# ekimb/rust-mdbg

Measured on AMD Instinct MI355X. Metric: Gbases/s ingested to k-min-mer graph, higher is better.
Workload: dtype u64

## Files before the change

### rust_mdbg_amd/csrc/table.hip

```cpp
#include "mdbg_dev.h"

struct __attribute__((aligned(32))) Slot {
    u64 word;
    u64 m1;
    u64 m2;
    u32 count;
    u32 pad;
};
constexpr u64 EMPTY = ~0ull;
constexpr u64 HMUL = 0x9E3779B97F4A7C15ull;

struct KeySrc {
    const u64* mh;
    const u64* arena;
    u32 k;
};

__device__ inline u64 load_relaxed(const u64* p) { return __hip_atomic_load(p, __ATOMIC_RELAXED, __HIP_MEMORY_SCOPE_AGENT); }

__device__ inline u64 rep_elem(const KeySrc& ks, u64 word, u32 j) {
    const u32 rep = (u32)word;
    if (word & (1ull << 33)) return ks.arena[(u64)rep * (ks.k + 2) + j];
    return (word & (1ull << 32)) ? ks.mh[(u64)rep + ks.k - 1 - j] : ks.mh[(u64)rep + j];
}

__device__ inline bool window_reversed(const u64* __restrict__ w, u32 k) {
    for (u32 j = 0; j < k / 2 + 1 && j < k; ++j) {
        const u64 a = w[j], b = w[k - 1 - j];
        if (a < b) return false;
        if (a > b) return true;
    }
    return true;
}
template <class ElemFn>
__device__ inline u64 key_hash_fn(ElemFn elem, u32 k) {
    u64 h0 = 0x243F6A8885A308D3ull, h1 = 0x13198A2E03707344ull, h2 = 0xA4093822299F31D0ull, h3 = 0x082EFA98EC4E6C89ull;
    u32 j = 0;
    for (; j + 4 <= k; j += 4) {
        h0 = (h0 ^ elem(j)) * HMUL;     h0 ^= h0 >> 29;
        h1 = (h1 ^ elem(j + 1)) * HMUL; h1 ^= h1 >> 29;
        h2 = (h2 ^ elem(j + 2)) * HMUL; h2 ^= h2 >> 29;
        h3 = (h3 ^ elem(j + 3)) * HMUL; h3 ^= h3 >> 29;
    }
    if (j < k) { h0 = (h0 ^ elem(j)) * HMUL; h0 ^= h0 >> 29; }
    if (j + 1 < k) { h1 = (h1 ^ elem(j + 1)) * HMUL; h1 ^= h1 >> 29; }
    if (j + 2 < k) { h2 = (h2 ^ elem(j + 2)) * HMUL; h2 ^= h2 >> 29; }
    return fmix64(h0 ^ rol64(h1, 17) ^ rol64(h2, 31) ^ rol64(h3, 47));
}
__device__ inline u64 key_hash_window(const u64* __restrict__ w, u32 k, bool rev) {
    return key_hash_fn([&](u32 j) { return rev ? w[k - 1 - j] : w[j]; }, k);
}
__device__ inline u64 key_hash_window_hbm(const u64* __restrict__ w, u32 k, bool rev, u64& smallest) {
    u64 h[4] = {0x243F6A8885A308D3ull, 0x13198A2E03707344ull, 0xA4093822299F31D0ull, 0x082EFA98EC4E6C89ull};
    const u64* const p = rev ? w + (k - 1) : w;
    const long st = rev ? -1 : 1;
    u64 mn = ~0ull;
    for (u32 j0 = 0; j0 < k; j0 += 16) {
        u64 v[16];
#pragma unroll
        for (int t = 0; t < 16; ++t) { const u32 j = j0 + t < k ? j0 + t : k - 1; v[t] = p[st * (long)j]; }
#pragma unroll
        for (int t = 0; t < 16; ++t)
            if (j0 + t < k) { h[t & 3] = (h[t & 3] ^ v[t]) * HMUL; h[t & 3] ^= h[t & 3] >> 29; mn = v[t] < mn ? v[t] : mn; }
    }
    smallest = mn;
    return fmix64(h[0] ^ rol64(h[1], 17) ^ rol64(h[2], 31) ^ rol64(h[3], 47));
}
__device__ inline u64 key_hash_canon(const u64* __restrict__ key, u32 k) {
    return key_hash_fn([&](u32 j) { return key[j]; }, k);
}

struct TableArgs {
    Slot* tab; u64 cap;
    u64* mx;
    u32 A;
    u64* n_distinct;
    KeySrc ks;
    u32 own_world, own_rank;
    const u64* own_thr;
    u32* probe_err;
    u64* own_inserted;
    u64 fp_mask;
    unsigned long long* link_ctr;
    u32 no_chain;
    u8* claim;
};

__device__ inline u64 home_slot(u64 h, u64 cap) { return __umul64hi(h << 24, cap); }

__device__ inline void push_ordinal(const TableArgs& T, u64 s, u64 x) {
    Slot* e = T.tab + s;
    const u32 A = T.A;
    const u64* last = A == 1 ? &e->m1 : A == 2 ? &e->m2 : &T.mx[s * (A - 2) + (A - 3)];
    if (x > load_relaxed(last)) return;
    u64 carry = x;
    for (u32 lvl = 0; lvl < A && carry != EMPTY; ++lvl) {
        u64* m = lvl == 0 ? &e->m1 : lvl == 1 ? &e->m2 : &T.mx[s * (A - 2) + (lvl - 2)];
        const u64 old = atomicMin((unsigned long long*)m, (unsigned long long)carry);
        if (old > carry) carry = old;
    }
}

template <class EqFn>
__device__ inline u64 upsert_slot_from(const TableArgs& T, u64 h, u64 myword_lo, EqFn same_key, bool& claimed, u64 s, u64 probes);
template <class EqFn>
__device__ inline u64 upsert_slot(const TableArgs& T, u64 h, u64 myword_lo, EqFn same_key, bool& claimed) {
    return upsert_slot_from(T, h, myword_lo, same_key, claimed, home_slot(h, T.cap), 0);
}
template <class EqFn>
__device__ inline u64 upsert_slot_from(const TableArgs& T, u64 h, u64 myword_lo, EqFn same_key, bool& claimed, u64 s, u64 probes) {
    claimed = false;
    const u64 fp = (h >> 34) & T.fp_mask;
    const u64 myword = (fp << 34) | myword_lo;
    for (; probes <= T.cap; ++probes) {
        u64 w = load_relaxed(&T.tab[s].word);
        if (w == EMPTY) {
            const u64 old = atomicCAS((unsigned long long*)&T.tab[s].word, (unsigned long long)EMPTY, (unsigned long long)myword);
            if (old == EMPTY) { wave_agg_inc(T.n_distinct); claimed = true; return s; }
            w = old;
        }
        if ((w >> 34) == fp && same_key(w)) return s;
        s = s + 1 == T.cap ? 0 : s + 1;
    }
    *T.probe_err = 1;
    return ~0ull;
}
typedef u64 u64x2_a8 __attribute__((ext_vector_type(2), aligned(8)));
__device__ inline bool same_key_window(const KeySrc& ks, u64 w, const u64* wl, bool rev_mine) {
    const u32 k = ks.k, rep = (u32)w;
    const u64* rp; bool cross;
    if (w & (1ull << 33)) { rp = ks.arena + (u64)rep * (k + 2); cross = rev_mine; }
    else { rp = ks.mh + rep; cross = rev_mine != ((w & (1ull << 32)) != 0); }
    if (k < 8) {
        u64 diff = 0;
        for (u32 j = 0; j < k; ++j) diff |= rp[j] ^ wl[cross ? k - 1 - j : j];
        return !diff;
    }
    if (k >= 16) {
        for (u32 j = 0;; j += 16) {
            if (j + 16 > k) j = k - 16;
            u64x2_a8 a[8];
#pragma unroll
            for (int t = 0; t < 8; ++t) a[t] = *(const u64x2_a8*)(rp + j + 2 * t);
            u64 diff = 0;
            if (!cross) {
                const u64* m = wl + j;
#pragma unroll
                for (int t = 0; t < 8; ++t) diff |= (a[t].x ^ m[2 * t]) | (a[t].y ^ m[2 * t + 1]);
            } else {
                const u64* m = wl + (k - 16 - j);
#pragma unroll
                for (int t = 0; t < 8; ++t) diff |= (a[t].x ^ m[15 - 2 * t]) | (a[t].y ^ m[14 - 2 * t]);
            }
            if (diff) return false;
            if (j + 16 >= k) return true;
        }
    }
    for (u32 j = 0;; j += 8) {
        if (j + 8 > k) j = k - 8;
        const u64x2_a8 a0 = *(const u64x2_a8*)(rp + j), a1 = *(const u64x2_a8*)(rp + j + 2),
                       a2 = *(const u64x2_a8*)(rp + j + 4), a3 = *(const u64x2_a8*)(rp + j + 6);
        u64 diff;
        if (!cross) {
            const u64* m = wl + j;
            diff = (a0.x ^ m[0]) | (a0.y ^ m[1]) | (a1.x ^ m[2]) | (a1.y ^ m[3]) | (a2.x ^ m[4]) | (a2.y ^ m[5]) | (a3.x ^ m[6]) | (a3.y ^ m[7]);
        } else {
            const u64* m = wl + (k - 8 - j);
            diff = (a0.x ^ m[7]) | (a0.y ^ m[6]) | (a1.x ^ m[5]) | (a1.y ^ m[4]) | (a2.x ^ m[3]) | (a2.y ^ m[2]) | (a3.x ^ m[1]) | (a3.y ^ m[0]);
        }
        if (diff) return false;
        if (j + 8 >= k) return true;
    }
}

constexpr u32 OWNER_BINS = 65536, OWNER_THR_AT = 1, OWNER_TAB_AT = 64, OWNER_PARAM_WORDS = OWNER_TAB_AT + OWNER_BINS / 8;
struct OwnerSpec { u32 world; const u64* thr; };
__device__ inline u32 owner_of_min(u64 m, u32 k, OwnerSpec os);
__device__ inline u32 window_owner(const u64* __restrict__ w, u32 k, OwnerSpec os) {
    if (os.world <= 1) return 0;
    u64 m = w[0];
    for (u32 j = 1; j < k; ++j) { const u64 x = w[j]; m = x < m ? x : m; }
    return owner_of_min(m, k, os);
}
__device__ inline u32 owner_of_min(u64 m, u32 k, OwnerSpec os) {
    (void)k;
    if (os.world <= 1) return 0;
    if (!os.thr) return (u32)__umul64hi(fmix64(m), (u64)os.world);
    const u64 mul = os.thr[0];
    if (mul) {
        const u64 bin = __umul64hi(m, mul);
        const u32 o = ((const u8*)(os.thr + OWNER_TAB_AT))[bin < OWNER_BINS ? bin : OWNER_BINS - 1];
        return o < os.world ? o : os.world - 1;
    }
    const u64* const thr = os.thr + OWNER_THR_AT;
    u32 lo = 0, hi = os.world - 1;
    while (lo < hi) { const u32 mid = (lo + hi) >> 1; if (thr[mid] <= m) lo = mid + 1; else hi = mid; }
    return lo;
}
__global__ void owner_thresholds_kernel(double bound, u32 k, u32 world, u64* __restrict__ thr) {
    const u32 r = threadIdx.x + 1;
    if (threadIdx.x == 0) thr[0] = 0;
    thr += OWNER_THR_AT;
    if (r >= world) return;
    const double x = -expm1(log1p(-(double)r / (double)world) / (double)k);
    double v = x * bound;
    thr[r - 1] = v >= 18446744073709549568.0 ? ~0ull : (u64)v;
}
void launch_owner_thresholds(double bound, u32 k, u32 world, u64* thr, hipStream_t s) {
    if (world > 1) hipLaunchKernelGGL(owner_thresholds_kernel, dim3(1), dim3(64), 0, s, bound, k, world, thr);
}

struct OwnerCodes { u64 mul; const u64* thr; u32 world; };
__device__ inline OwnerCodes owner_codes_of(OwnerSpec os) { OwnerCodes c; c.thr = os.thr; c.world = os.world; c.mul = os.thr ? os.thr[0] : 0; return c; }
__device__ inline u16 owner_code(u64 v, const OwnerCodes& c) {
    if (c.mul) { const u64 bin = __umul64hi(v, c.mul); return (u16)(bin < OWNER_BINS ? bin : OWNER_BINS - 1); }
    const u64* const thr = c.thr + OWNER_THR_AT;
    u32 lo = 0, hi = c.world - 1;
    while (lo < hi) { const u32 mid = (lo + hi) >> 1; if (thr[mid] <= v) lo = mid + 1; else hi = mid; }
    return (u16)lo;
}
__device__ inline u32 owner_of_code(u16 code, const OwnerCodes& c) {
    if (!c.mul) return code;
    const u32 o = ((const u8*)(c.thr + OWNER_TAB_AT))[code];
    return o < c.world ? o : c.world - 1;
}
template <class ValueFn, class ValidFn>
__device__ inline const u16* span_min_codes(ValueFn value, ValidFn valid, u32 nv, u32 k, const OwnerCodes& c, u16* a, u16* b, u32& p) {
    for (u32 t = threadIdx.x; t < nv; t += 256) a[t] = valid(t) ? owner_code(value(t), c) : (u16)0xFFFFu;
    __syncthreads();
    for (p = 1; 2 * p <= k; p *= 2) {
        for (u32 t = threadIdx.x; t < nv; t += 256) { const u16 x = a[t], y = t + p < nv ? a[t + p] : (u16)0xFFFFu; b[t] = x < y ? x : y; }
        __syncthreads();
        u16* const sw = a; a = b; b = sw;
    }
    return a;
}

__device__ inline u64 upsert_wave_h(const TableArgs& T, bool act, u32 li, u64 i, const u64* w, u32 k, bool rev, u64 h, bool& claimed, bool& found);
__device__ inline u64 upsert_wave(const TableArgs& T, bool act, u32 li, u64 i, const u64* w, u32 k, bool& claimed, bool& found) {
    bool rev = false; u64 h = 0;
    if (act) { rev = window_reversed(w, k); h = key_hash_window(w, k, rev); }
    return upsert_wave_h(T, act, li, i, w, k, rev, h, claimed, found);
}
__device__ inline u64 upsert_wave_h(const TableArgs& T, bool act, u32 li, u64 i, const u64* w, u32 k, bool rev, u64 h, bool& claimed, bool& found) {
    const int lane = threadIdx.x & 63;
    const u64 fp = (h >> 34) & T.fp_mask;
    const u64 myword_lo = ((u64)rev << 32) | (u64)(u32)i;
    auto eq = [&](u64 word) { return same_key_window(T.ks, word, w, rev); };
    u64 s = act ? home_slot(h, T.cap) : 0, word = EMPTY, probes = 0;
    claimed = false;
    bool cand = false;
    if (act) {
        for (; probes <= T.cap; ++probes) {
            u64 wv = load_relaxed(&T.tab[s].word);
            if (wv == EMPTY) {
                const u64 old = atomicCAS((unsigned long long*)&T.tab[s].word, (unsigned long long)EMPTY, (unsigned long long)((fp << 34) | myword_lo));
                if (old == EMPTY) { wave_agg_inc(T.n_distinct); claimed = true; break; }
                wv = old;
            }
            if ((wv >> 34) == fp) { word = wv; cand = true; break; }
            s = s + 1 == T.cap ? 0 : s + 1;
        }
        if (!claimed && !cand) { *T.probe_err = 1; s = ~0ull; }
    }
    const bool cross = rev != ((word & (1ull << 32)) != 0);
    const u32 rep = (u32)word;
    const u32 p_li = (u32)__shfl_up((int)li, 1, 64), p_rep = (u32)__shfl_up((int)rep, 1, 64);
    const int p_info = __shfl_up((int)((cand && !(word & (1ull << 33)) ? 1 : 0) | (cross ? 2 : 0)), 1, 64);
    const bool link = cand && !T.no_chain && lane > 0 && !(word & (1ull << 33)) && (p_info & 1) && p_li + 1 == li && ((p_info >> 1) & 1) == (int)cross &&
                      rep == (cross ? p_rep - 1u : p_rep + 1u);
    bool pass = false;
    if (cand) pass = link ? T.ks.mh[(u64)rep + (cross ? 0u : k - 1u)] == w[k - 1] : eq(word);
    const u64 heads = __ballot(!link), fails = __ballot(cand && !pass);
    found = pass;
    if (link && pass) {
        const int hp = 63 - __clzll((unsigned long long)(heads & ((2ull << lane) - 1ull)));
        found = ((fails >> hp) & ((2ull << (lane - hp)) - 1ull)) == 0;
    }
    if (T.link_ctr) { const u64 lm = __ballot(link && found); if (lane == 0 && lm) atomicAdd(T.link_ctr, (unsigned long long)__popcll(lm)); }
    if (cand && !found) {
        const bool skip = !link;
        s = upsert_slot_from(T, h, myword_lo, eq, claimed, skip ? (s + 1 == T.cap ? 0 : s + 1) : s, probes + (skip ? 1 : 0));
        found = !claimed && s != ~0ull;
    }
    return s;
}

constexpr int OWN_SPAN = 2048;
__global__ __launch_bounds__(256) void insert_windows_kernel(TableArgs T, const u64* __restrict__ mh, const u32* __restrict__ mread,
                                                                   const u64* __restrict__ roff, u64 i0, u64 i1, u32 slot0, u64 first_ordinal,
                                                                   u32* __restrict__ cap_err, const u64* __restrict__ i1_dev, u64 n_lim) {
    extern __shared__ u64 sh_keys[];
    if (cap_err[1]) return;
    if (i1_dev) { i1 = *i1_dev; if (i0 + (u64)blockIdx.x * OWN_SPAN >= i1) return; }
    const u32 k = T.ks.k;
    u16* const list = (u16*)(sh_keys + OWN_SPAN + k);
    u32* const n_own = (u32*)(list + OWN_SPAN);
    u8* const cl = (u8*)(n_own + 4);
    const u64 b0 = i0 + (u64)blockIdx.x * OWN_SPAN;
    const u64 lim = b0 + OWN_SPAN + k - 1 < i1 ? b0 + OWN_SPAN + k - 1 : i1;
    for (u64 t = b0 + threadIdx.x; t < lim; t += 256) sh_keys[t - b0] = mh[t];
    if (threadIdx.x == 0) *n_own = 0;
    if (T.claim) for (int u = threadIdx.x; u < OWN_SPAN / 8; u += 256) ((u64*)cl)[u] = 0;
    __syncthreads();
    const bool by_codes = T.own_world > 1 && T.own_thr != nullptr;
    const u16* mc = nullptr; u32 pc = 1; OwnerCodes oc{};
    if (by_codes) {
        u16* const ca = (u16*)(cl + OWN_SPAN);
        oc = owner_codes_of(OwnerSpec{T.own_world, T.own_thr});
        const u32 n_st = (u32)(lim - b0);
        mc = span_min_codes([&](u32 t) { return sh_keys[t]; }, [&](u32 t) { return t < n_st; }, OWN_SPAN + k - 1, k, oc, ca, ca + (OWN_SPAN + k), pc);
    }
#pragma unroll
    for (int u = 0; u < OWN_SPAN / 256; ++u) {
        const u32 li = u * 256 + threadIdx.x;
        const u64 i = b0 + li;
        bool mine = false;
        bool own = i + k <= i1;
        if (own && T.own_world > 1) {
            if (by_codes) { const u16 x = mc[li], y = mc[li + k - pc]; own = owner_of_code(x < y ? x : y, oc) == T.own_rank; }
            else own = window_owner(sh_keys + li, k, OwnerSpec{T.own_world, T.own_thr}) == T.own_rank;
        }
        if (own) {
            const u32 slot = mread[i];
            const u64 rs = roff[slot], re = roff[slot + 1];
            mine = re - rs > k && i + k <= re;
        }
        const u64 m = __ballot(mine);
        u32 base = 0;
        if ((threadIdx.x & 63) == 0 && m) base = atomicAdd(n_own, (u32)__popcll(m));
        base = __shfl(base, 0, 64);
        if (mine) list[base + __popcll(m & ((1ull << (threadIdx.x & 63)) - 1))] = (u16)li;
    }
    __syncthreads();
    const u32 n = *n_own;
    if (threadIdx.x == 0 && n && T.own_world > 1) atomicAdd((unsigned long long*)ctr_shard(T.own_inserted), (unsigned long long)n);
    for (u32 j0 = 0; j0 < n; j0 += 256) {
        const u32 j = j0 + threadIdx.x;
        bool act = j < n;
        const u32 li = act ? list[j] : 0u;
        const u64 i = b0 + li;
        u64 ord = 0;
        if (act) {
            const u32 slot = mread[i];
            const u64 win = i - roff[slot];
            if (win > WIN_MASK) { *cap_err = 1; act = false; }
            ord = ((first_ordinal + (slot - slot0)) << WIN_BITS) | win;
        }
        bool claimed, found;
        const u64 s = upsert_wave(T, act, li, i, sh_keys + li, k, claimed, found);
        if (claimed && T.claim) cl[li] = 1;
        if (found) {
            atomicAdd(&T.tab[s].count, 1u);
            push_ordinal(T, s, ord);
        }
    }
    if (T.claim) {
        __syncthreads();
        const u64 hi = i1 - b0 < (u64)OWN_SPAN ? i1 - b0 : (u64)OWN_SPAN;
        for (u32 li = threadIdx.x; li < hi && li < n_lim - (u64)blockIdx.x * OWN_SPAN; li += 256) T.claim[b0 + li] = cl[li];
    }
}

constexpr int OWNL_SPAN = 2048;
constexpr u32 OWNL_MAX_WORLD = 64;
struct OwnerBases { u64 b[OWNL_MAX_WORLD]; };
__device__ inline bool window_starts_at(const u32* __restrict__ mread, const u64* __restrict__ roff, u64 i, u64 i1, u32 k) {
    if (i >= i1) return false;
    const u32 slot = mread[i];
    const u64 rs = roff[slot], re = roff[slot + 1];
    return re - rs > k && i + k <= re;
}
constexpr u32 OWNL_LDS_MAX_K = 1024;
__global__ __launch_bounds__(256) void owner_bins_kernel(const u64* __restrict__ mh, const u32* __restrict__ mread, const u64* __restrict__ roff, u64 i0, u64 i1, u32 k, u64 mul,
                                                         unsigned long long* __restrict__ hist) {
    extern __shared__ u64 sh_min[];
    const u64 b0 = i0 + (u64)blockIdx.x * OWNL_SPAN;
    const bool staged = k <= OWNL_LDS_MAX_K;
    OwnerCodes oc{}; oc.mul = mul;
    const u16* cur = nullptr; u32 p = 1;
    if (staged) { u16* const ca = (u16*)sh_min; cur = span_min_codes([&](u32 t) { return mh[b0 + t]; }, [&](u32 t) { return b0 + t < i1; }, OWNL_SPAN + k - 1, k, oc, ca, ca + (OWNL_SPAN + k), p); }
    const int lane = threadIdx.x & 63;
#pragma unroll 1
    for (int u = 0; u < OWNL_SPAN / 256; ++u) {
        const u32 li = u * 256 + threadIdx.x;
        const u64 i = b0 + li;
        u32 bin = 0xFFFFFFFFu;
        if (window_starts_at(mread, roff, i, i1, k)) {
            if (staged) { const u16 x = cur[li], y = cur[li + k - p]; bin = x < y ? x : y; }
            else { u64 m = mh[i]; for (u32 j = 1; j < k; ++j) { const u64 x = mh[i + j]; m = x < m ? x : m; } bin = owner_code(m, oc); }
        }
        for (u64 todo = __ballot(bin != 0xFFFFFFFFu); todo;) {
            const u32 bb = (u32)__shfl((int)bin, __ffsll((unsigned long long)todo) - 1, 64);
            const u64 mm = __ballot(bin == bb);
            if (bin == bb && (mm & ((1ull << lane) - 1)) == 0) atomicAdd(&hist[bb], (unsigned long long)__popcll(mm));
            todo &= ~mm;
        }
    }
}
void launch_owner_bins(const u64* mh, const u32* mread, const u64* roff, u64 i0, u64 i1, u32 k, u64 mul, u64* hist, hipStream_t s) {
    const size_t lds = k <= OWNL_LDS_MAX_K ? 2 * ((size_t)OWNL_SPAN + k) * sizeof(u16) : 0;
    if (i1 > i0) hipLaunchKernelGGL(owner_bins_kernel, dim3((unsigned)((i1 - i0 + OWNL_SPAN - 1) / OWNL_SPAN)), dim3(256), lds, s, mh, mread, roff, i0, i1, k, mul, (unsigned long long*)hist);
}
__global__ __launch_bounds__(256) void owner_list_count_kernel(const u64* __restrict__ mh, const u32* __restrict__ mread, const u64* __restrict__ roff, u64 i0, u64 i1,
                                                               u32 k, u32 world, const u64* thr, u32* __restrict__ blk_cnt, u8* __restrict__ owner_of) {
    extern __shared__ u64 sh_min[];
    __shared__ u32 hist[OWNL_MAX_WORLD];
    if (threadIdx.x < world) hist[threadIdx.x] = 0;
    const u64 b0 = i0 + (u64)blockIdx.x * OWNL_SPAN;
    const OwnerSpec os{world, thr};
    const bool staged = k <= OWNL_LDS_MAX_K && thr != nullptr && world > 1;
    OwnerCodes oc{}; const u16* cur = nullptr; u32 p = 1;
    if (staged) {
        oc = owner_codes_of(os);
        u16* const ca = (u16*)sh_min;
        cur = span_min_codes([&](u32 t) { return mh[b0 + t]; }, [&](u32 t) { return b0 + t < i1; }, OWNL_SPAN + k - 1, k, oc, ca, ca + (OWNL_SPAN + k), p);
    } else __syncthreads();
#pragma unroll
    for (int u = 0; u < OWNL_SPAN / 256; ++u) {
        const u32 li = u * 256 + threadIdx.x;
        const u64 i = b0 + li;
        u32 o = 0xFFu;
        if (window_starts_at(mread, roff, i, i1, k)) {
            if (staged) { const u16 x = cur[li], y = cur[li + k - p]; o = owner_of_code(x < y ? x : y, oc); }
            else o = window_owner(mh + i, k, os);
            atomicAdd(&hist[o], 1u);
        }
        if (i < i1) owner_of[i - i0] = (u8)o;
    }
    __syncthreads();
    if (threadIdx.x < world) blk_cnt[(size_t)blockIdx.x * world + threadIdx.x] = hist[threadIdx.x];
}
__global__ __launch_bounds__(256) void owner_list_write_kernel(const u64* __restrict__ mh, const u32* __restrict__ mread, const u64* __restrict__ roff, u64 i0, u64 i1,
                                                               u32 k, u32 world, const u64* thr, u32 slot0, const u64* __restrict__ blk_off, OwnerBases bases, u32* __restrict__ list,
                                                               const u8* __restrict__ owner_of, u32 direct_owner, u32* __restrict__ direct_dst) {
    constexpr int NG = OWNL_SPAN / 64;
    __shared__ u32 grp[NG][OWNL_MAX_WORLD];
    for (int t = threadIdx.x; t < NG * (int)OWNL_MAX_WORLD; t += 256) ((u32*)grp)[t] = 0;
    __syncthreads();
    const u64 b0 = i0 + (u64)blockIdx.x * OWNL_SPAN;
    const int lane = threadIdx.x & 63, wv = threadIdx.x >> 6;
    constexpr u32 NONE = 0xFFFFFFFFu;
    u32 own[OWNL_SPAN / 256], rank[OWNL_SPAN / 256], slot_of[OWNL_SPAN / 256];
#pragma unroll
    for (int u = 0; u < OWNL_SPAN / 256; ++u) {
        const u64 i = b0 + u * 256 + threadIdx.x;
        u32 o = NONE, slot = 0;
        if (i < i1) { const u32 ob = owner_of[i - i0]; if (ob != 0xFFu) { o = ob; slot = mread[i]; } }
        u32 r = 0;
        for (u64 todo = __ballot(o != NONE); todo;) {
            const u32 oo = (u32)__shfl((int)o, __ffsll((unsigned long long)todo) - 1, 64);
            const u64 m = __ballot(o == oo);
            if (o == oo) { r = (u32)__popcll(m & ((1ull << lane) - 1)); if (r == 0) grp[u * 4 + wv][oo] = (u32)__popcll(m); }
            todo &= ~m;
        }
        own[u] = o; rank[u] = r; slot_of[u] = slot;
    }
    __syncthreads();
    if (threadIdx.x < world) { u32 run = 0; for (int g = 0; g < NG; ++g) { const u32 c = grp[g][threadIdx.x]; grp[g][threadIdx.x] = run; run += c; } }
    __syncthreads();
#pragma unroll
    for (int u = 0; u < OWNL_SPAN / 256; ++u) {
        const u32 o = own[u];
        if (o == NONE || (o == direct_owner && !direct_dst)) continue;
        const u64 i = b0 + u * 256 + threadIdx.x;
        const u64 at = blk_off[(size_t)blockIdx.x * world + o] + grp[u * 4 + wv][o] + rank[u];
        uint2* const e = o == direct_owner ? (uint2*)direct_dst + at : (uint2*)list + (bases.b[o] + at);
        *e = make_uint2((u32)(i - i0), slot_of[u] - slot0);
    }
}

struct SegBuckets { u64 start[OWNL_MAX_WORLD + 1]; u64 base[OWNL_MAX_WORLD]; u64 lim[OWNL_MAX_WORLD]; u32 n; u32 skip; };
__device__ inline u32 seg_bucket_of(const SegBuckets& B, u64 j) {
    u32 lo = 0, hi = B.n - 1;
    while (lo < hi) { const u32 mid = (lo + hi + 1) >> 1; if (B.start[mid] <= j) lo = mid; else hi = mid - 1; }
    return lo;
}
__device__ inline u32 seg_add_of(const uint2* __restrict__ list, u64 j, u32 k, const SegBuckets& B, u32& b) {
    b = seg_bucket_of(B, j);
    if (b == B.skip) return 0;
    if (j && B.start[b] != j) { const u32 d = list[j].x - list[j - 1].x; if (d < k) return d; }
    return k;
}
constexpr u32 SEG_BLOCK = 4096;
__global__ __launch_bounds__(256) void seg_sums_kernel(const uint2* __restrict__ list, u64 n, u32 k, SegBuckets B, u64* __restrict__ block_sum) {
    __shared__ u32 ws[4];
    u32 v = 0;
#pragma unroll
    for (int q = 0; q < SEG_BLOCK / 256; ++q) { const u64 j = (u64)blockIdx.x * SEG_BLOCK + q * 256 + threadIdx.x; u32 b; if (j < n) v += seg_add_of(list, j, k, B, b); }
    for (int d = 32; d; d >>= 1) v += __shfl_down(v, d, 64);
    if ((threadIdx.x & 63) == 0) ws[threadIdx.x >> 6] = v;
    __syncthreads();
    if (threadIdx.x == 0) block_sum[blockIdx.x] = (u64)ws[0] + ws[1] + ws[2] + ws[3];
}
__global__ __launch_bounds__(256) void seg_pick_kernel(const uint2* __restrict__ list, u64 n, u32 k, SegBuckets B, const u64* __restrict__ block_base, const u64* __restrict__ total,
                                                       u64* __restrict__ out) {
    __shared__ u32 ws[4];
    const u32 bq = blockIdx.x;
    const u64 j1 = bq < B.n ? B.start[bq] : n;
    if (j1 >= n) { if (threadIdx.x == 0) out[bq] = total[0]; return; }
    const u64 j0 = j1 - j1 % SEG_BLOCK;
    u32 v = 0;
#pragma unroll
    for (int q = 0; q < SEG_BLOCK / 256; ++q) { const u64 j = j0 + q * 256 + threadIdx.x; u32 b; if (j < j1) v += seg_add_of(list, j, k, B, b); }
    for (int d = 32; d; d >>= 1) v += __shfl_down(v, d, 64);
    if ((threadIdx.x & 63) == 0) ws[threadIdx.x >> 6] = v;
    __syncthreads();
    if (threadIdx.x == 0) out[bq] = block_base[j0 / SEG_BLOCK] + ws[0] + ws[1] + ws[2] + ws[3];
}
__global__ __launch_bounds__(256) void seg_copy_kernel(const uint2* __restrict__ list, u64 n, u32 k, SegBuckets B, const u64* __restrict__ block_base,
                                                       u64* __restrict__ store, u64* __restrict__ payload, u64 payload_n, u32 to_store) {
    __shared__ u32 lpre[256];
    __shared__ u64 laddr[256];
    __shared__ u32 tmp[8];
    u64 P0 = block_base[blockIdx.x];
#pragma unroll 1
    for (int q = 0; q < SEG_BLOCK / 256; ++q) {
        const u64 j = (u64)blockIdx.x * SEG_BLOCK + q * 256 + threadIdx.x;
        u32 a = 0, b = 0, x = 0;
        if (j < n) { a = seg_add_of(list, j, k, B, b); x = list[j].x; }
        u32 T;
        const u32 excl = block_excl_scan_256(a, tmp, T);
        u64 at = ~0ull;
        if (j < n && !((u64)x + k > B.lim[b] || P0 + excl + a > payload_n)) at = B.base[b] + x + (k - a);
        lpre[threadIdx.x] = j < n ? excl : 0xFFFFFFFFu;
        laddr[threadIdx.x] = at;
        __syncthreads();
        for (u32 e = threadIdx.x; e < T; e += 256) {
            u32 lo = 0, hi = 255;
#pragma unroll
            for (int st = 0; st < 8; ++st) { const u32 mid = (lo + hi + 1) >> 1; if (lpre[mid] <= e) lo = mid; else hi = mid - 1; }
            const u64 src = laddr[lo];
            if (src == ~0ull) continue;
            u64* const h = store + src + (e - lpre[lo]);
            u64* const pp = payload + P0 + e;
            if (to_store) *h = *pp; else *pp = *h;
        }
        P0 += T;
    }
}
__device__ inline bool listed_check(u64 j) { return (((u32)j * 0x9E3779B1u) >> 28) == 0; }
struct ListedBatch { u64 start, m0, m1, first_ordinal; const u32* list; u32 slot0, n_reads; };
__global__ __launch_bounds__(256) void insert_listed_entries_kernel(TableArgs T, const u64* __restrict__ mh, u32* __restrict__ mread, const u64* __restrict__ roff,
                                                                    u64 m0, u64 m1, const u32* __restrict__ list, u64 n, u32 slot0, u32 n_reads, u64 first_ordinal,
                                                                    u32* __restrict__ cap_err, const ListedBatch* __restrict__ multi, u32 n_multi) {
    if (cap_err[1]) return;
    const u64 j = (u64)blockIdx.x * blockDim.x + threadIdx.x;
    const u32 k = T.ks.k;
    bool ok = j < n;
    u64 i = 0, rs = 0; u32 slot = 0;
    u64 jl = j;
    if (multi) {
        const u64 jw0 = (u64)blockIdx.x * blockDim.x + (threadIdx.x & ~63u);
        u64 jw = ((u64)__builtin_amdgcn_readfirstlane((u32)(jw0 >> 32)) << 32) | (u64)__builtin_amdgcn_readfirstlane((u32)jw0);
        if (jw >= n) jw = n - 1;
        u32 lo = 0, hi = n_multi - 1;
        while (lo < hi) { const u32 mid = (lo + hi + 1) >> 1; if (multi[mid].start <= jw) lo = mid; else hi = mid - 1; }
        if (ok && multi[lo + 1].start <= j) {
            hi = n_multi - 1;
            while (lo < hi) { const u32 mid = (lo + hi + 1) >> 1; if (multi[mid].start <= j) lo = mid; else hi = mid - 1; }
        }
        const ListedBatch b = multi[lo];
        m0 = b.m0; m1 = b.m1; list = b.list; slot0 = b.slot0; n_reads = b.n_reads; first_ordinal = b.first_ordinal; jl = j - b.start;
    }
    if (ok) {
        const uint2 e = ((const uint2*)list)[jl];
        i = m0 + e.x; slot = slot0 + e.y; ok = e.y < n_reads && i + k <= m1;
    }
    const u64* const w = mh + i;
    bool rev = false; u64 h = 0;
    if (ok) {
        const u64 w_first = w[0], w_last = w[k - 1];
        rs = roff[slot]; const u64 re = roff[slot + 1];
        ok = i >= rs && re - rs > k && i + k <= re;
        if (ok) {
            rev = w_first != w_last ? w_first > w_last : window_reversed(w, k);
            u64 smallest;
            h = key_hash_window_hbm(w, k, rev, smallest);
            ok = owner_of_min(smallest, k, OwnerSpec{T.own_world, T.own_thr}) == T.own_rank;
        }
    }
    wave_count_add(ok, T.own_inserted);
    const u64 win = i - rs;
    if (ok && win > WIN_MASK) { *cap_err = 1; ok = false; }
    const u64 ord = ((first_ordinal + (slot - slot0)) << WIN_BITS) | win;
    bool claimed, found;
    const u64 s = upsert_wave_h(T, ok, (u32)i, i, w, k, rev, h, claimed, found);
    if (claimed) { mread[i] = slot; if (T.claim) T.claim[i] = 1; }
    if (found) {
        atomicAdd(&T.tab[s].count, 1u);
        push_ordinal(T, s, ord);
    }
}
__global__ __launch_bounds__(256) void list_segments_kernel(const u32* __restrict__ list, u64 n, u32 n_spans, u32* __restrict__ seg) {
    const u64 j = (u64)blockIdx.x * blockDim.x + threadIdx.x;
    if (j >= n) return;
    const u32 last = n_spans - 1;
    u32 b = list[2 * j] / OWNL_SPAN; if (b > last) b = last;
    int pb = -1;
    if (j) { u32 q = list[2 * j - 2] / OWNL_SPAN; if (q > last) q = last; pb = (int)q; }
    for (int q = pb + 1; q <= (int)b; ++q) seg[q] = (u32)j;
}
__global__ __launch_bounds__(256) void insert_listed_span_kernel(TableArgs T, const u64* __restrict__ mh, u32* __restrict__ mread, const u64* __restrict__ roff,
                                                                 u64 m0, u64 m1, const u32* __restrict__ list, const u32* __restrict__ seg, u64 n, u32 slot0,
                                                                 u32 n_reads, u64 first_ordinal, u32* __restrict__ cap_err) {
    extern __shared__ u64 sh_keys[];
    if (cap_err[1]) return;
    const u32 q = blockIdx.x, k = T.ks.k;
    const u32 s0 = seg[q], s1 = seg[q + 1];
    const u64 b0 = m0 + (u64)q * OWNL_SPAN;
    u8* const cl = (u8*)(sh_keys + OWNL_SPAN + k);
    const u64 span_n = m1 - b0 < (u64)OWNL_SPAN ? m1 - b0 : (u64)OWNL_SPAN;
    if (s0 >= s1 || s1 > n) {
        if (T.claim) for (u32 li = threadIdx.x; li < span_n; li += 256) T.claim[b0 + li] = 0;
        return;
    }
    const u64 lim = b0 + OWNL_SPAN + k - 1 < m1 ? b0 + OWNL_SPAN + k - 1 : m1;
    for (u64 t = b0 + threadIdx.x; t < lim; t += 256) sh_keys[t - b0] = mh[t];
    if (T.claim) for (int u = threadIdx.x; u < OWNL_SPAN / 8; u += 256) ((u64*)cl)[u] = 0;
    __syncthreads();
    for (u32 base = s0; base < s1; base += 256) {
        const u32 j = base + threadIdx.x;
        bool ok = j < s1;
        u32 li = 0; u64 i = 0;
        u32 slot = 0; u64 rs = 0;
        if (ok) {
            const uint2 e = ((const uint2*)list)[j];
            li = e.x; ok = li / OWNL_SPAN == q && e.y < n_reads; li -= q * OWNL_SPAN; i = b0 + li; slot = slot0 + e.y;
        }
        if (ok) {
            rs = roff[slot]; const u64 re = roff[slot + 1];
            ok = i >= rs && re - rs > k && i + k <= re && (!listed_check(j) || window_owner(sh_keys + li, k, OwnerSpec{T.own_world, T.own_thr}) == T.own_rank);
        }
        wave_count_add(ok, T.own_inserted);
        const u64 win = i - rs;
        if (ok && win > WIN_MASK) { *cap_err = 1; ok = false; }
        const u64 ord = ((first_ordinal + (slot - slot0)) << WIN_BITS) | win;
        bool claimed, found;
        const u64 s = upsert_wave(T, ok, li, i, sh_keys + li, k, claimed, found);
        if (claimed) { mread[i] = slot; if (T.claim) cl[li] = 1; }
        if (found) {
            atomicAdd(&T.tab[s].count, 1u);
            push_ordinal(T, s, ord);
        }
    }
    if (T.claim) {
        __syncthreads();
        for (u32 li = threadIdx.x; li < span_n; li += 256) T.claim[b0 + li] = cl[li];
    }
}
u32 owner_list_spans(u64 n_minimizers) { return (u32)((n_minimizers + OWNL_SPAN - 1) / OWNL_SPAN); }
void launch_list_segments(const u32* list, u64 n, u32 n_spans, u32* seg, hipStream_t s) {
    (void)hipMemsetD32Async((hipDeviceptr_t)seg, (int)(u32)n, (size_t)n_spans + 1, s);
    if (n && n_spans) hipLaunchKernelGGL(list_segments_kernel, dim3((unsigned)((n + 255) / 256)), dim3(256), 0, s, list, n, n_spans, seg);
}
void launch_owner_list_count(const u64* mh, const u32* mread, const u64* roff, u64 i0, u64 i1, u32 k, u32 world, const u64* thr, u32* blk_cnt, u8* owner_of, hipStream_t s) {
    const size_t lds = k <= OWNL_LDS_MAX_K ? 2 * ((size_t)OWNL_SPAN + k) * sizeof(u16) : 0;
    if (i1 > i0) hipLaunchKernelGGL(owner_list_count_kernel, dim3((unsigned)((i1 - i0 + OWNL_SPAN - 1) / OWNL_SPAN)), dim3(256), lds, s, mh, mread, roff, i0, i1, k, world, thr, blk_cnt, owner_of);
}
void launch_owner_list_write(const u64* mh, const u32* mread, const u64* roff, u64 i0, u64 i1, u32 k, u32 world, const u64* thr, u32 slot0, const u64* blk_off, const OwnerBases& bases, u32* list, const u8* owner_of, hipStream_t s,
                             u32 direct_owner = 0xFFFFFFFFu, u32* direct_dst = nullptr) {
    if (i1 > i0) hipLaunchKernelGGL(owner_list_write_kernel, dim3((unsigned)((i1 - i0 + OWNL_SPAN - 1) / OWNL_SPAN)), dim3(256), 0, s, mh, mread, roff, i0, i1, k, world, thr, slot0, blk_off, bases, list, owner_of, direct_owner, direct_dst);
}
static void launch_listed_entries(const TableArgs& T, const u64* mh, u32* mread, const u64* roff, u64 m0, u64 m1, const u32* list, u64 n, u32 slot0, u32 n_reads, u64 first_ordinal,
                                  u32* cap_err, const ListedBatch* multi, u32 n_multi, hipStream_t s) {
    hipLaunchKernelGGL(insert_listed_entries_kernel, dim3((unsigned)((n + 255) / 256)), dim3(256), 0, s, T, mh, mread, roff, m0, m1, list, n, slot0, n_reads, first_ordinal, cap_err, multi, n_multi);
}
constexpr u64 LISTED_SPAN_MIN = 150;
static size_t listed_span_lds(const TableArgs& T) { return ((size_t)OWNL_SPAN + T.ks.k) * sizeof(u64) + OWNL_SPAN; }
bool listed_per_entry(const TableArgs& T, u64 m0, u64 m1, u64 n, bool have_seg) {
    return !have_seg || listed_span_lds(T) > 64 * 1024 || n < (u64)owner_list_spans(m1 - m0) * LISTED_SPAN_MIN;
}
void launch_insert_listed(const TableArgs& T, const u64* mh, u32* mread, const u64* roff, u64 m0, u64 m1, const u32* list, const u32* seg, u64 n, u32 slot0,
                          u32 n_reads, u64 first_ordinal, u32* cap_err, hipStream_t s) {
    if (!n) return;
    if (!listed_per_entry(T, m0, m1, n, seg != nullptr))
        hipLaunchKernelGGL(insert_listed_span_kernel, dim3(owner_list_spans(m1 - m0)), dim3(256), listed_span_lds(T), s, T, mh, mread, roff, m0, m1, list, seg, n, slot0, n_reads, first_ordinal, cap_err);
    else
        launch_listed_entries(T, mh, mread, roff, m0, m1, list, n, slot0, n_reads, first_ordinal, cap_err, nullptr, 0u, s);
}
void launch_insert_listed_multi(const TableArgs& T, const u64* mh, u32* mread, const u64* roff, const ListedBatch* d_batches, u32 n_batches, u64 total, u32* cap_err, hipStream_t s) {
    if (!total) return;
    launch_listed_entries(T, mh, mread, roff, 0ull, 0ull, nullptr, total, 0u, 0u, 0ull, cap_err, d_batches, n_batches, s);
}

__global__ __launch_bounds__(256) void reserve_check_kernel(const u64* __restrict__ distinct_shards, u64* __restrict__ n_distinct, const u64* __restrict__ batch_windows, u64 cap,
                                                            u32* __restrict__ too_small, const u64* __restrict__ carry, u64 store_cap, const u32* __restrict__ over_max) {
    __shared__ u64 ws[4];
    u64 v = 0;
    for (int i = threadIdx.x; i < CTR_SHARDS; i += 256) v += distinct_shards[i];
    for (int d = 32; d; d >>= 1) v += __shfl_down(v, d, 64);
    if ((threadIdx.x & 63) == 0) ws[threadIdx.x >> 6] = v;
    __syncthreads();
    if (threadIdx.x == 0) {
        const u64 nd = ws[0] + ws[1] + ws[2] + ws[3];
        *n_distinct = nd;
        const u64 n = nd + *batch_windows;
        bool skip = n + n / 2 + 1024 > cap;
        if (carry) skip = skip || *carry > store_cap || *carry >= 0xFFFFFFF0ull || (over_max && *over_max);
        *too_small = skip ? 1u : 0u;
    }
}

__global__ __launch_bounds__(1024) void count_reserve_kernel(const u64* __restrict__ roff, u32 slot0, u32 n_reads, u32 k, u64* __restrict__ batch_windows, u32* __restrict__ done,
                                                             const u64* __restrict__ distinct_shards, u64* __restrict__ n_distinct, u64 cap, u32* __restrict__ too_small,
                                                             const u64* __restrict__ carry, u64 store_cap, const u32* __restrict__ over_max) {
    __shared__ u64 ws[16];
    __shared__ u32 last;
    u64 w = 0;
    for (u32 r = blockIdx.x * blockDim.x + threadIdx.x; r < n_reads; r += gridDim.x * blockDim.x) { const u64 n = roff[slot0 + r + 1] - roff[slot0 + r]; if (n > k) w += n - k + 1; }
    for (int d = 32; d; d >>= 1) w += __shfl_down(w, d, 64);
    if ((threadIdx.x & 63) == 0) ws[threadIdx.x >> 6] = w;
    __syncthreads();
    if (threadIdx.x == 0) {
        u64 t = 0;
        for (int i = 0; i < 16; ++i) t += ws[i];
        if (t) atomicAdd((unsigned long long*)batch_windows, (unsigned long long)t);
        __threadfence();
        last = atomicAdd(done, 1u) + 1u == gridDim.x ? 1u : 0u;
    }
    __syncthreads();
    if (!last) return;
    __threadfence();
    u64 v = 0;
    for (int i = threadIdx.x; i < CTR_SHARDS; i += 1024) v += distinct_shards[i];
    for (int d = 32; d; d >>= 1) v += __shfl_down(v, d, 64);
    __syncthreads();
    if ((threadIdx.x & 63) == 0) ws[threadIdx.x >> 6] = v;
    __syncthreads();
    if (threadIdx.x == 0) {
        u64 nd = 0;
        for (int i = 0; i < 16; ++i) nd += ws[i];
        *n_distinct = nd;
        const u64 bw = __hip_atomic_load(batch_windows, __ATOMIC_RELAXED, __HIP_MEMORY_SCOPE_AGENT);
        const u64 n = nd + bw;
        bool skip = n + n / 2 + 1024 > cap;
        if (carry) skip = skip || *carry > store_cap || *carry >= 0xFFFFFFF0ull || (over_max && *over_max);
        *too_small = skip ? 1u : 0u;
        *done = 0;
    }
}
void launch_count_reserve(const u64* roff, u32 slot0, u32 n_reads, u32 k, u64* batch_windows, u32* done, const u64* distinct_shards, u64* n_distinct, u64 cap, u32* too_small,
                          const u64* carry, u64 store_cap, const u32* over_max, hipStream_t s) {
    hipLaunchKernelGGL(count_reserve_kernel, dim3(n_reads ? std::min<u32>(64u, (n_reads + 1023) / 1024) : 1), dim3(1024), 0, s, roff, slot0, n_reads, k, batch_windows, done, distinct_shards, n_distinct, cap,
                       too_small, carry, store_cap, over_max);
}

__global__ __launch_bounds__(256) void insert_records_kernel(TableArgs T, u64 r0, u64 r1, u64* __restrict__ n_windows) {
    const u64 r = r0 + (u64)blockIdx.x * blockDim.x + threadIdx.x;
    if (r >= r1) return;
    const u32 k = T.ks.k;
    const u64* key = T.ks.arena + r * (k + 2);
    const u64 h = key[k + 1];
    bool claimed;
    const u64 s = upsert_slot(T, h, (1ull << 33) | (u64)(u32)r, [&](u64 word) { return same_key_window(T.ks, word, key, false); }, claimed);
    if (claimed || s == ~0ull) return;
    atomicAdd(&T.tab[s].count, 1u);
    push_ordinal(T, s, key[k]);
    (void)n_windows;
}

struct ZeroList { u64* p[6]; u64 n[6]; u64* set_p; u64 set_v; };
__global__ void clear_table_kernel(Slot* __restrict__ tab, u64 cap, u64* __restrict__ mx, u64 n_mx, ZeroList z) {
    const u64 stride = (u64)gridDim.x * blockDim.x;
    {
        const u64 i0 = (u64)blockIdx.x * blockDim.x + threadIdx.x;
#pragma unroll
        for (int r = 0; r < 6; ++r) for (u64 i = i0; i < z.n[r]; i += stride) z.p[r][i] = 0;
        if (i0 == 0 && z.set_p) *z.set_p = z.set_v;
    }
    for (u64 i = (u64)blockIdx.x * blockDim.x + threadIdx.x; i < cap; i += stride) {
        uint4* p = (uint4*)(tab + i);
        p[0] = make_uint4(0xFFFFFFFFu, 0xFFFFFFFFu, 0xFFFFFFFFu, 0xFFFFFFFFu);
        p[1] = make_uint4(0xFFFFFFFFu, 0xFFFFFFFFu, 0u, 0u);
    }
    for (u64 i = (u64)blockIdx.x * blockDim.x + threadIdx.x; i < n_mx; i += stride) mx[i] = EMPTY;
}

__global__ void rehash_kernel(const Slot* __restrict__ old, u64 old_cap, const u64* __restrict__ old_mx, TableArgs T) {
    const u64 i = (u64)blockIdx.x * blockDim.x + threadIdx.x;
    if (i >= old_cap) return;
    const Slot e = old[i];
    if (e.word == EMPTY) return;
    const u64 h = key_hash_fn([&](u32 j) { return rep_elem(T.ks, e.word, j); }, T.ks.k);
    u64 s = home_slot(h, T.cap);
    for (;;) {
        const u64 oldw = atomicCAS((unsigned long long*)&T.tab[s].word, (unsigned long long)EMPTY, (unsigned long long)e.word);
        if (oldw == EMPTY) break;
        s = s + 1 == T.cap ? 0 : s + 1;
    }
    T.tab[s].m1 = e.m1; T.tab[s].m2 = e.m2; T.tab[s].count = e.count;
    for (u32 j = 0; j + 2 < T.A; ++j) T.mx[s * (T.A - 2) + j] = old_mx[i * (T.A - 2) + j];
}

struct BatchTab {
    const u64* first_ordinal; const u32* n_reads; const u32* slot0; const u64* rank_base; u32 n;
    const u32* by_slot0; const u64* by_slot_first;
    const u64* by_m0; const u64* by_m0_rank;
    const u64* m0;
};
struct FinArgs {
    const Slot* tab; u64 cap; const u64* mx; u32 A; u32 casc; u32 k; u32 l;
    const u64* mh; const u32* mpos; const u64* roff; const u32* mread; const u64* arena;
    BatchTab bt;
    u64* solid_list; u64* solid_count;
    u64* solid_dense;
    const u64* n_solid_dev;
    const u64* order;
    u64* o_row;
    const u64* ath_override;
    u64* bm_first; u64* bm_solid;
    u32 claims;
    u8* by_first; u8* by_solid;
    const u32* pre_first; const u32* pre_solid;
    u64* sh_solid; u64* sh_wrapped; u64* sh_distinct;
    u64* o_keys; u32* o_index; u16* o_abund; u32* o_seqlen; u16* o_shift; u64* o_shift_full;
    u64* o_src_read; u64* o_src_start; u64* o_src_end; u8* o_rev;
};

__device__ inline void decode_ordinal(const FinArgs& F, u64 ord, u64& i, u64& D) {
    const u64 ro = ord >> WIN_BITS, win = ord & WIN_MASK;
    u32 lo = 0, hi = F.bt.n - 1;
    while (lo < hi) { const u32 mid = lo + ((hi - lo + 1) >> 1); if (F.bt.first_ordinal[mid] <= ro) lo = mid; else hi = mid - 1; }
    const u32 s0 = F.bt.slot0[lo];
    const u32 slot = s0 + (u32)(ro - F.bt.first_ordinal[lo]);
    i = F.roff[slot] + win;
    D = F.bt.rank_base[lo] + (i - F.roff[s0]);
}
__device__ inline u64 dense_of_index(const FinArgs& F, u64 i) {
    u32 lo = 0, hi = F.bt.n - 1;
    while (lo < hi) { const u32 mid = lo + ((hi - lo + 1) >> 1); if (F.bt.by_m0[mid] <= i) lo = mid; else hi = mid - 1; }
    return F.bt.by_m0_rank[lo] + (i - F.bt.by_m0[lo]);
}
__device__ inline u64 rep_ordinal(const FinArgs& F, u64 word) {
    const u32 rep = (u32)word;
    if (word & (1ull << 33)) return F.arena[(u64)rep * (F.k + 2) + F.k];
    const u32 slot = F.mread[rep];
    u32 lo = 0, hi = F.bt.n - 1;
    while (lo < hi) { const u32 mid = lo + ((hi - lo + 1) >> 1); if (F.bt.by_slot0[mid] <= slot) lo = mid; else hi = mid - 1; }
    return ((F.bt.by_slot_first[lo] + (slot - F.bt.by_slot0[lo])) << WIN_BITS) | ((u64)rep - F.roff[slot]);
}
struct SlotView { u32 count; u64 first, ath; bool solid; };
__device__ inline SlotView slot_view(const Slot& e, u64 s, const u64* mx, u32 casc, u32 A_filter, u64 r, const u64* ath_override = nullptr) {
    SlotView v;
    v.count = e.count + 1u;
    v.first = r < e.m1 ? r : e.m1;
    const u32 A = casc;
    if (A == 1) v.ath = v.first;
    else {
        const u64 prev = A == 2 ? e.m1 : A == 3 ? e.m2 : mx[s * (A - 2) + (A - 4)];
        const u64 last = A == 2 ? e.m2 : mx[s * (A - 2) + (A - 3)];
        v.ath = r < prev ? prev : (r < last ? r : last);
    }
    v.solid = A_filter == 1 || (u16)v.count >= (u16)A_filter;
    if (e.pad && ath_override) v.ath = ath_override[e.pad - 1];
    return v;
}

constexpr int FIN_SPT = 4;
__global__ __launch_bounds__(1024) void fin_mark_kernel(FinArgs F) {
    __shared__ u32 wcnt[16 * FIN_SPT];
    __shared__ u64 bbase;
    const u64 s0 = (u64)blockIdx.x * (1024 * FIN_SPT) + threadIdx.x;
    Slot e[FIN_SPT];
#pragma unroll
    for (int u = 0; u < FIN_SPT; ++u) { const u64 s = s0 + 1024ull * u; e[u].word = EMPTY; if (s < F.cap) e[u] = F.tab[s]; }
    u32 n_occ = 0, n_wrapped = 0; bool solid[FIN_SPT]; u64 m[FIN_SPT], dense[FIN_SPT];
    const int lane = threadIdx.x & 63, wv = threadIdx.x >> 6;
#pragma unroll
    for (int u = 0; u < FIN_SPT; ++u) {
        solid[u] = false;
        u64 D = 0;
        if (e[u].word != EMPTY) {
            const u32 count = e[u].count + 1u;
            ++n_occ; solid[u] = F.A == 1 || (u16)count >= (u16)F.A; n_wrapped += count >= 65536u ? 1u : 0u;
            if (e[u].word & (1ull << 33)) { u64 i; const u64 ro = rep_ordinal(F, e[u].word); decode_ordinal(F, ro < e[u].m1 ? ro : e[u].m1, i, D); }
            else {
                D = dense_of_index(F, (u32)e[u].word);
                if (e[u].count) { u64 i, D1; decode_ordinal(F, e[u].m1, i, D1); if (D1 < D) D = D1; }
            }
            F.by_first[D] = 1;
            if (solid[u]) F.by_solid[D] = 1;
        }
        dense[u] = D;
        m[u] = __ballot(solid[u]);
        if (lane == 0) wcnt[16 * u + wv] = (u32)__popcll(m[u]);
    }
    for (int d = 32; d; d >>= 1) { n_occ += __shfl_down(n_occ, d, 64); n_wrapped += __shfl_down(n_wrapped, d, 64); }
    if (lane == 0) {
        if (n_occ) atomicAdd((unsigned long long*)ctr_shard(F.sh_distinct), (unsigned long long)n_occ);
        if (n_wrapped) atomicAdd((unsigned long long*)ctr_shard(F.sh_wrapped), (unsigned long long)n_wrapped);
    }
    __syncthreads();
    if (threadIdx.x == 0) {
        u32 tot = 0;
        for (int i = 0; i < 16 * FIN_SPT; ++i) { const u32 c = wcnt[i]; wcnt[i] = tot; tot += c; }
        bbase = tot ? atomicAdd((unsigned long long*)F.solid_count, (unsigned long long)tot) : 0;
    }
    __syncthreads();
#pragma unroll
    for (int u = 0; u < FIN_SPT; ++u)
        if (solid[u]) {
            const u64 j = bbase + wcnt[16 * u + wv] + __popcll(m[u] & ((1ull << lane) - 1));
            F.solid_list[j] = s0 + 1024ull * u; F.solid_dense[j] = dense[u];
        }
}
__global__ __launch_bounds__(1024) void fin_mark_claims_kernel(FinArgs F) {
    constexpr u32 SPAN = 1024 * FIN_SPT;
    __shared__ u16 lst[SPAN], sol_li[SPAN];
    __shared__ u32 sol_D[SPAN];
    __shared__ u32 n_lst, n_sol;
// ... 690 lines not shown
```

Baseline: 2510.

## Prefetch slot minimum during probe, merge count+ordinal update, and software-pipeline read offsets

The hash-table probe now loads the slot's last-ordinal threshold alongside the slot word, so the early-exit check in the sighting update needs no separate dependent load after key comparison. The count increment and first atomicMin are issued back to back in a merged add_sighting routine. The key-compare routine is rewritten as a generic grouped loop issuing up to three 8-word groups of loads before comparing. In one insert kernel the mread/roff lookups for the next iteration are prefetched to hide latency. This adds extra loads on every probe step (including mismatched slots) and uses a possibly stale threshold, which is safe since atomicMin chain still enforces ordering.

```diff
diff --git a/rust_mdbg_amd/csrc/table.hip b/rust_mdbg_amd/csrc/table.hip
--- a/rust_mdbg_amd/csrc/table.hip
+++ b/rust_mdbg_amd/csrc/table.hip
@@ -88,44 +88,53 @@
 
 __device__ inline u64 home_slot(u64 h, u64 cap) { return __umul64hi(h << 24, cap); }
 
-__device__ inline void push_ordinal(const TableArgs& T, u64 s, u64 x) {
+__device__ inline u64 slot_last_near(const TableArgs& T, u64 s) { return load_relaxed(T.A == 1 ? &T.tab[s].m1 : &T.tab[s].m2); }
+__device__ inline u64 slot_last_far(const TableArgs& T, u64 s, u64 near) { return T.A <= 2 ? near : load_relaxed(&T.mx[s * (T.A - 2) + (T.A - 3)]); }
+__device__ inline void add_sighting(const TableArgs& T, u64 s, u64 x, u64 last) {
     Slot* e = T.tab + s;
     const u32 A = T.A;
-    const u64* last = A == 1 ? &e->m1 : A == 2 ? &e->m2 : &T.mx[s * (A - 2) + (A - 3)];
-    if (x > load_relaxed(last)) return;
-    u64 carry = x;
-    for (u32 lvl = 0; lvl < A && carry != EMPTY; ++lvl) {
-        u64* m = lvl == 0 ? &e->m1 : lvl == 1 ? &e->m2 : &T.mx[s * (A - 2) + (lvl - 2)];
+    if (x > last) { atomicAdd(&e->count, 1u); return; }
+    const u64 first = atomicMin((unsigned long long*)&e->m1, (unsigned long long)x);
+    atomicAdd(&e->count, 1u);
+    u64 carry = first > x ? first : x;
+    for (u32 lvl = 1; lvl < A && carry != EMPTY; ++lvl) {
+        u64* m = lvl == 1 ? &e->m2 : &T.mx[s * (A - 2) + (lvl - 2)];
         const u64 old = atomicMin((unsigned long long*)m, (unsigned long long)carry);
         if (old > carry) carry = old;
     }
 }
 
 template <class EqFn>
-__device__ inline u64 upsert_slot_from(const TableArgs& T, u64 h, u64 myword_lo, EqFn same_key, bool& claimed, u64 s, u64 probes);
+__device__ inline u64 upsert_slot_from(const TableArgs& T, u64 h, u64 myword_lo, EqFn same_key, bool& claimed, u64& last, u64 s, u64 probes);
 template <class EqFn>
-__device__ inline u64 upsert_slot(const TableArgs& T, u64 h, u64 myword_lo, EqFn same_key, bool& claimed) {
-    return upsert_slot_from(T, h, myword_lo, same_key, claimed, home_slot(h, T.cap), 0);
+__device__ inline u64 upsert_slot(const TableArgs& T, u64 h, u64 myword_lo, EqFn same_key, bool& claimed, u64& last) {
+    return upsert_slot_from(T, h, myword_lo, same_key, claimed, last, home_slot(h, T.cap), 0);
 }
 template <class EqFn>
-__device__ inline u64 upsert_slot_from(const TableArgs& T, u64 h, u64 myword_lo, EqFn same_key, bool& claimed, u64 s, u64 probes) {
+__device__ inline u64 upsert_slot_from(const TableArgs& T, u64 h, u64 myword_lo, EqFn same_key, bool& claimed, u64& last, u64 s, u64 probes) {
     claimed = false;
     const u64 fp = (h >> 34) & T.fp_mask;
     const u64 myword = (fp << 34) | myword_lo;
     for (; probes <= T.cap; ++probes) {
         u64 w = load_relaxed(&T.tab[s].word);
+        const u64 near = slot_last_near(T, s);
         if (w == EMPTY) {
             const u64 old = atomicCAS((unsigned long long*)&T.tab[s].word, (unsigned long long)EMPTY, (unsigned long long)myword);
             if (old == EMPTY) { wave_agg_inc(T.n_distinct); claimed = true; return s; }
             w = old;
         }
-        if ((w >> 34) == fp && same_key(w)) return s;
+        if ((w >> 34) == fp) {
+            last = slot_last_far(T, s, near);
+            if (same_key(w)) return s;
+        }
         s = s + 1 == T.cap ? 0 : s + 1;
     }
     *T.probe_err = 1;
     return ~0ull;
 }
 typedef u64 u64x2_a8 __attribute__((ext_vector_type(2), aligned(8)));
+constexpr int CMP_GROUPS_INSERT = 3;
+template <int G = 2>
 __device__ inline bool same_key_window(const KeySrc& ks, u64 w, const u64* wl, bool rev_mine) {
     const u32 k = ks.k, rep = (u32)w;
     const u64* rp; bool cross;
@@ -136,41 +145,33 @@
         for (u32 j = 0; j < k; ++j) diff |= rp[j] ^ wl[cross ? k - 1 - j : j];
         return !diff;
     }
-    if (k >= 16) {
-        for (u32 j = 0;; j += 16) {
-            if (j + 16 > k) j = k - 16;
-            u64x2_a8 a[8];
-#pragma unroll
-            for (int t = 0; t < 8; ++t) a[t] = *(const u64x2_a8*)(rp + j + 2 * t);
-            u64 diff = 0;
-            if (!cross) {
-                const u64* m = wl + j;
-#pragma unroll
-                for (int t = 0; t < 8; ++t) diff |= (a[t].x ^ m[2 * t]) | (a[t].y ^ m[2 * t + 1]);
-            } else {
-                const u64* m = wl + (k - 16 - j);
-#pragma unroll
-                for (int t = 0; t < 8; ++t) diff |= (a[t].x ^ m[15 - 2 * t]) | (a[t].y ^ m[14 - 2 * t]);
+    for (u32 j0 = 0; j0 < k; j0 += 8 * G) {
+        u64x2_a8 a[G][4];
+#pragma unroll
+        for (int g = 0; g < G; ++g)
+            if (j0 + 8 * g < k) {
+                const u32 j = j0 + 8 * g + 8 <= k ? j0 + 8 * g : k - 8;
+#pragma unroll
+                for (int t = 0; t < 4; ++t) a[g][t] = *(const u64x2_a8*)(rp + j + 2 * t);
             }
-            if (diff) return false;
-            if (j + 16 >= k) return true;
-        }
-    }
-    for (u32 j = 0;; j += 8) {
-        if (j + 8 > k) j = k - 8;
-        const u64x2_a8 a0 = *(const u64x2_a8*)(rp + j), a1 = *(const u64x2_a8*)(rp + j + 2),
-                       a2 = *(const u64x2_a8*)(rp + j + 4), a3 = *(const u64x2_a8*)(rp + j + 6);
-        u64 diff;
-        if (!cross) {
-            const u64* m = wl + j;
-            diff = (a0.x ^ m[0]) | (a0.y ^ m[1]) | (a1.x ^ m[2]) | (a1.y ^ m[3]) | (a2.x ^ m[4]) | (a2.y ^ m[5]) | (a3.x ^ m[6]) | (a3.y ^ m[7]);
-        } else {
-            const u64* m = wl + (k - 8 - j);
-            diff = (a0.x ^ m[7]) | (a0.y ^ m[6]) | (a1.x ^ m[5]) | (a1.y ^ m[4]) | (a2.x ^ m[3]) | (a2.y ^ m[2]) | (a3.x ^ m[1]) | (a3.y ^ m[0]);
-        }
+        u64 diff = 0;
+#pragma unroll
+        for (int g = 0; g < G; ++g)
+            if (j0 + 8 * g < k) {
+                const u32 j = j0 + 8 * g + 8 <= k ? j0 + 8 * g : k - 8;
+                if (!cross) {
+                    const u64* m = wl + j;
+#pragma unroll
+                    for (int t = 0; t < 4; ++t) diff |= (a[g][t].x ^ m[2 * t]) | (a[g][t].y ^ m[2 * t + 1]);
+                } else {
+                    const u64* m = wl + (k - 8 - j);
+#pragma unroll
+                    for (int t = 0; t < 4; ++t) diff |= (a[g][t].x ^ m[7 - 2 * t]) | (a[g][t].y ^ m[6 - 2 * t]);
+                }
+            }
         if (diff) return false;
-        if (j + 8 >= k) return true;
-    }
+    }
+    return true;
 }
 
 constexpr u32 OWNER_BINS = 65536, OWNER_THR_AT = 1, OWNER_TAB_AT = 64, OWNER_PARAM_WORDS = OWNER_TAB_AT + OWNER_BINS / 8;
@@ -236,29 +237,30 @@
     return a;
 }
 
-__device__ inline u64 upsert_wave_h(const TableArgs& T, bool act, u32 li, u64 i, const u64* w, u32 k, bool rev, u64 h, bool& claimed, bool& found);
-__device__ inline u64 upsert_wave(const TableArgs& T, bool act, u32 li, u64 i, const u64* w, u32 k, bool& claimed, bool& found) {
+__device__ inline u64 upsert_wave_h(const TableArgs& T, bool act, u32 li, u64 i, const u64* w, u32 k, bool rev, u64 h, bool& claimed, bool& found, u64& last);
+__device__ inline u64 upsert_wave(const TableArgs& T, bool act, u32 li, u64 i, const u64* w, u32 k, bool& claimed, bool& found, u64& last) {
     bool rev = false; u64 h = 0;
     if (act) { rev = window_reversed(w, k); h = key_hash_window(w, k, rev); }
-    return upsert_wave_h(T, act, li, i, w, k, rev, h, claimed, found);
-}
-__device__ inline u64 upsert_wave_h(const TableArgs& T, bool act, u32 li, u64 i, const u64* w, u32 k, bool rev, u64 h, bool& claimed, bool& found) {
+    return upsert_wave_h(T, act, li, i, w, k, rev, h, claimed, found, last);
+}
+__device__ inline u64 upsert_wave_h(const TableArgs& T, bool act, u32 li, u64 i, const u64* w, u32 k, bool rev, u64 h, bool& claimed, bool& found, u64& last) {
     const int lane = threadIdx.x & 63;
     const u64 fp = (h >> 34) & T.fp_mask;
     const u64 myword_lo = ((u64)rev << 32) | (u64)(u32)i;
-    auto eq = [&](u64 word) { return same_key_window(T.ks, word, w, rev); };
+    auto eq = [&](u64 word) { return same_key_window<CMP_GROUPS_INSERT>(T.ks, word, w, rev); };
     u64 s = act ? home_slot(h, T.cap) : 0, word = EMPTY, probes = 0;
-    claimed = false;
+    claimed = false; last = 0;
     bool cand = false;
     if (act) {
         for (; probes <= T.cap; ++probes) {
             u64 wv = load_relaxed(&T.tab[s].word);
+            const u64 near = slot_last_near(T, s);
             if (wv == EMPTY) {
                 const u64 old = atomicCAS((unsigned long long*)&T.tab[s].word, (unsigned long long)EMPTY, (unsigned long long)((fp << 34) | myword_lo));
                 if (old == EMPTY) { wave_agg_inc(T.n_distinct); claimed = true; break; }
                 wv = old;
             }
-            if ((wv >> 34) == fp) { word = wv; cand = true; break; }
+            if ((wv >> 34) == fp) { word = wv; cand = true; last = slot_last_far(T, s, near); break; }
             s = s + 1 == T.cap ? 0 : s + 1;
         }
         if (!claimed && !cand) { *T.probe_err = 1; s = ~0ull; }
@@ -280,7 +282,7 @@
     if (T.link_ctr) { const u64 lm = __ballot(link && found); if (lane == 0 && lm) atomicAdd(T.link_ctr, (unsigned long long)__popcll(lm)); }
     if (cand && !found) {
         const bool skip = !link;
-        s = upsert_slot_from(T, h, myword_lo, eq, claimed, skip ? (s + 1 == T.cap ? 0 : s + 1) : s, probes + (skip ? 1 : 0));
+        s = upsert_slot_from(T, h, myword_lo, eq, claimed, last, skip ? (s + 1 == T.cap ? 0 : s + 1) : s, probes + (skip ? 1 : 0));
         found = !claimed && s != ~0ull;
     }
     return s;
@@ -335,25 +337,28 @@
     __syncthreads();
     const u32 n = *n_own;
     if (threadIdx.x == 0 && n && T.own_world > 1) atomicAdd((unsigned long long*)ctr_shard(T.own_inserted), (unsigned long long)n);
+    u32 slot_n = 0; u64 rs_n = 0;
+    if (threadIdx.x < n) { slot_n = mread[b0 + list[threadIdx.x]]; rs_n = roff[slot_n]; }
     for (u32 j0 = 0; j0 < n; j0 += 256) {
         const u32 j = j0 + threadIdx.x;
         bool act = j < n;
         const u32 li = act ? list[j] : 0u;
         const u64 i = b0 + li;
+        const u32 slot = slot_n;
+        const u64 rs = rs_n;
+        const bool act_n = j + 256 < n;
+        if (act_n) slot_n = mread[b0 + list[j + 256]];
         u64 ord = 0;
         if (act) {
-            const u32 slot = mread[i];
-            const u64 win = i - roff[slot];
+            const u64 win = i - rs;
             if (win > WIN_MASK) { *cap_err = 1; act = false; }
             ord = ((first_ordinal + (slot - slot0)) << WIN_BITS) | win;
         }
-        bool claimed, found;
-        const u64 s = upsert_wave(T, act, li, i, sh_keys + li, k, claimed, found);
+        bool claimed, found; u64 last;
+        const u64 s = upsert_wave(T, act, li, i, sh_keys + li, k, claimed, found, last);
+        if (act_n) rs_n = roff[slot_n];
         if (claimed && T.claim) cl[li] = 1;
-        if (found) {
-            atomicAdd(&T.tab[s].count, 1u);
-            push_ordinal(T, s, ord);
-        }
+        if (found) add_sighting(T, s, ord, last);
     }
     if (T.claim) {
         __syncthreads();
@@ -584,13 +589,10 @@
     const u64 win = i - rs;
     if (ok && win > WIN_MASK) { *cap_err = 1; ok = false; }
     const u64 ord = ((first_ordinal + (slot - slot0)) << WIN_BITS) | win;
-    bool claimed, found;
-    const u64 s = upsert_wave_h(T, ok, (u32)i, i, w, k, rev, h, claimed, found);
+    bool claimed, found; u64 last;
+    const u64 s = upsert_wave_h(T, ok, (u32)i, i, w, k, rev, h, claimed, found, last);
     if (claimed) { mread[i] = slot; if (T.claim) T.claim[i] = 1; }
-    if (found) {
-        atomicAdd(&T.tab[s].count, 1u);
-        push_ordinal(T, s, ord);
-    }
+    if (found) add_sighting(T, s, ord, last);
 }
 __global__ __launch_bounds__(256) void list_segments_kernel(const u32* __restrict__ list, u64 n, u32 n_spans, u32* __restrict__ seg) {
     const u64 j = (u64)blockIdx.x * blockDim.x + threadIdx.x;
@@ -636,13 +638,10 @@
         const u64 win = i - rs;
         if (ok && win > WIN_MASK) { *cap_err = 1; ok = false; }
         const u64 ord = ((first_ordinal + (slot - slot0)) << WIN_BITS) | win;
-        bool claimed, found;
-        const u64 s = upsert_wave(T, ok, li, i, sh_keys + li, k, claimed, found);
+        bool claimed, found; u64 last;
+        const u64 s = upsert_wave(T, ok, li, i, sh_keys + li, k, claimed, found, last);
         if (claimed) { mread[i] = slot; if (T.claim) cl[li] = 1; }
-        if (found) {
-            atomicAdd(&T.tab[s].count, 1u);
-            push_ordinal(T, s, ord);
-        }
+        if (found) add_sighting(T, s, ord, last);
     }
     if (T.claim) {
         __syncthreads();
@@ -752,11 +751,10 @@
     const u32 k = T.ks.k;
     const u64* key = T.ks.arena + r * (k + 2);
     const u64 h = key[k + 1];
-    bool claimed;
-    const u64 s = upsert_slot(T, h, (1ull << 33) | (u64)(u32)r, [&](u64 word) { return same_key_window(T.ks, word, key, false); }, claimed);
+    bool claimed; u64 last = 0;
+    const u64 s = upsert_slot(T, h, (1ull << 33) | (u64)(u32)r, [&](u64 word) { return same_key_window<CMP_GROUPS_INSERT>(T.ks, word, key, false); }, claimed, last);
     if (claimed || s == ~0ull) return;
-    atomicAdd(&T.tab[s].count, 1u);
-    push_ordinal(T, s, key[k]);
+    add_sighting(T, s, key[k], last);
     (void)n_windows;
 }
 
```

New measurement: 2491. Within noise of the previous version (-0.7%).
